# ds2-lab/LambdaFS

Hardware: AMD Instinct MI355X
Metric: RS encode+decode GiB/s device-resident; 1/2/4/8 MI355X; %HBM roofline (higher is better)
Workload: dtype u8; 1 GPU; RS(10,4) encode + 1-erasure decode (data shard 0), 1024 KiB cells, 1024 stripes/GPU, device-resident; encodeBulk / decodeBulk via hrs_encode_dev / hrs_decode_dev; stripes_per_gpu=1024, stripes_total=1024, cell_bytes=1048576, k=10, p=4, parallelism=stripe-sharded x1 (RCCL: matrix broadcast + barriers only)

## Files before the change

include/hrs.h:

```cpp
#ifndef HRS_H_
#define HRS_H_

#include <stddef.h>
#include <stdint.h>

#ifdef __cplusplus
extern "C" {
#endif

typedef int hrs_status;
enum {
  HRS_OK = 0,
  HRS_EINVAL = 1,
  HRS_ETOOMANY = 2,
  HRS_EDEVICE = 3,
  HRS_ENOMEM = 4,
  HRS_EALIGN = 5
};

typedef struct hrs_codec hrs_codec;

enum {
  HRS_CODE_RS = 0,
  HRS_CODE_XOR = 1,
// ... 7 lines not shown
  int device;
  int reserved[7];
} hrs_opts;


hrs_status hrs_create(int stripe_size, int parity_size, const hrs_opts* opts, hrs_codec** out);
hrs_status hrs_create_code(int code, int stripe_size, int parity_size, const hrs_opts* opts,
                           hrs_codec** out);
int hrs_code_kind(const hrs_codec* codec);
hrs_status hrs_create_src(int stripe_size, int parity_size, int src_parity_size, const hrs_opts* opts,
                          hrs_codec** out);
hrs_status hrs_src_layout(const hrs_codec* codec, int* src_parities, int* rs_parities, int* group_degree);
void hrs_destroy(hrs_codec* codec);
const char* hrs_last_error(const hrs_codec* codec);
const char* hrs_last_kernel(const hrs_codec* codec);
const char* hrs_last_host_path(const hrs_codec* codec);
const char* hrs_version(void);


int hrs_device_count(void);
int hrs_codec_device(const hrs_codec* codec);

int hrs_stripe_size(const hrs_codec* codec);
int hrs_parity_size(const hrs_codec* codec);
int hrs_symbol_size(const hrs_codec* codec);


hrs_status hrs_locations_to_read_list(const hrs_codec* codec, const int* erased, int num_erased, int* to_read,
                                      int* num_to_read);

// ... 122 lines not shown
```

lambdafs_amd/_lib.py:

```python
import ctypes
import os

try:
    import torch
except ImportError:
    torch = None

_HERE = os.path.dirname(os.path.abspath(__file__))
LIB_PATH = os.environ.get("HRS_LIB") or os.path.join(_HERE, "libhrs.so")
PROBE_LIB_PATH = os.path.join(_HERE, "libhrs_probe.so")

HRS_OK = 0
HRS_EINVAL = 1
HRS_ETOOMANY = 2
HRS_EDEVICE = 3
HRS_ENOMEM = 4
HRS_EALIGN = 5

HRS_CODE_RS = 0
HRS_CODE_XOR = 1
HRS_CODE_NRS = 2
HRS_CODE_SRC = 3

EXPORTS = (
    "hrs_create", "hrs_create_code", "hrs_create_src", "hrs_src_layout", "hrs_code_kind", "hrs_destroy",
    "hrs_last_error", "hrs_version", "hrs_locations_to_read_list",
    "hrs_stripe_size", "hrs_parity_size", "hrs_symbol_size",
    "hrs_locations_to_read", "hrs_encode_matrix", "hrs_decode_matrix",
    "hrs_encode", "hrs_decode", "hrs_decode3", "hrs_encode_crc", "hrs_decode_crc",
    "hrs_encode_dev", "hrs_decode_dev", "hrs_decode_batch_dev", "hrs_apply_dev", "hrs_crc32_dev",
    "hrs_encode_crc_dev", "hrs_decode_crc_dev", "hrs_decode_batch_host", "hrs_encode_batch_host",
    "hrs_encode_submit", "hrs_decode_submit", "hrs_collect", "hrs_pending", "hrs_ticket_shape",
    "hrs_set_kernel_mode", "hrs_last_kernel", "hrs_wait", "hrs_release",
    "hrs_device_count", "hrs_codec_device", "hrs_decode_batch_host_multi", "hrs_encode_batch_host_multi",
    "hrs_set_timing", "hrs_ticket_gpu_ms", "hrs_last_host_path",
    "hrs_compute_error_locations", "hrs_scrub_dev", "hrs_scrub_batch_host",
    "hrs_heal_dev", "hrs_heal_batch_host", "hrs_heal_host",
)
PROBE_EXPORTS = ("hrs_probe_stream", "hrs_probe_rows")


class HrsError(IOError):

    def __init__(self, status, msg):
        super().__init__(f"hrs status {status}: {msg}")
        self.status = status


class HipOpts(ctypes.Structure):
    _fields_ = [("device", ctypes.c_int), ("reserved", ctypes.c_int * 7)]


# ... 46 lines not shown
        "hrs_encode_batch_host_multi": ([PP, I, P, S, S, S, S], I),
        "hrs_device_count": ([], I),
        "hrs_set_timing": ([P, I], I),
        "hrs_ticket_gpu_ms": ([P, ctypes.c_uint64, ctypes.POINTER(ctypes.c_float)], I),
        "hrs_codec_device": ([P], I),
        "hrs_encode_submit": ([P, PP, S, I, ctypes.POINTER(ctypes.c_uint64)], I),
        "hrs_decode_submit": ([P, PP, IP, I, IP, I, IP, I, S, I, ctypes.POINTER(ctypes.c_uint64)], I),
        "hrs_collect": ([P, ctypes.c_uint64, PP, P], I),
        "hrs_pending": ([P], I),
        "hrs_wait": ([P, ctypes.c_uint64], I),
        "hrs_release": ([P, ctypes.c_uint64], I),
        "hrs_ticket_shape": ([P, ctypes.c_uint64, IP, ctypes.POINTER(ctypes.c_size_t), IP], I),
        "hrs_set_kernel_mode": ([P, I], I),
        "hrs_last_kernel": ([P], ctypes.c_char_p),
        "hrs_last_host_path": ([P], ctypes.c_char_p),
        "hrs_compute_error_locations": ([P, IP, IP, IP, IP], I),
        "hrs_scrub_dev": ([P, PP, S, S, S, P, S, P], I),
        "hrs_scrub_batch_host": ([P, P, S, S, S, S, P, S], I),
        "hrs_heal_dev": ([P, PP, S, S, S, P, S, P], I),
        "hrs_heal_batch_host": ([P, P, S, S, S, S, P, S], I),
        "hrs_heal_host": ([P, PP, S, P], I),
    }
    for name, (args, res) in sigs.items():
        f = getattr(L, name)
        f.argtypes = args
        f.restype = res
    _lib = L
    return L


# ... 39 lines not shown
```

lambdafs_amd/csrc/hrs_api.cpp:

```cpp
#include <hip/hip_runtime.h>

#include <algorithm>
#include <cstdio>
#include <cstring>
#include <map>
#include <string>
#include <vector>

#include "../../include/hrs.h"
#include "hrs_codec.hpp"
#include <cstdarg>

#include "gf256.hpp"

namespace hrs::api {

namespace gf = hrs::gf;

thread_local std::string g_create_error;

hrs_status fail(hrs_codec* c, hrs_status st, const char* fmt, ...) {
  char buf[512];
  va_list ap;
  va_start(ap, fmt);
// ... 118 lines not shown
  if (group_degree) *group_degree = c->src_d;
  return HRS_OK;
}

void hrs_destroy(hrs_codec* c) {
  if (!c) return;
  if (c->device == HRS_DEVICE_NONE) {
    delete c;
    return;
  }
  DeviceGuard g(c->device);
  if (c->stream) {
    (void)hipStreamSynchronize(c->stream);
    (void)hipStreamDestroy(c->stream);
  }
  if (c->crc_tables_a) (void)hipFree(c->crc_tables_a);
  for (auto& kv : c->crc_fold_tables) {
    for (auto& u : kv.second.uses) {
      (void)hipEventSynchronize(u.ev);
      (void)hipEventDestroy(u.ev);
    }
    (void)hipFree(kv.second.dev);
  }
  if (c->crc_raw_done) {
    (void)hipEventSynchronize(c->crc_raw_done);
    (void)hipEventDestroy(c->crc_raw_done);
  }
  if (c->crc_raw) (void)hipFree(c->crc_raw);
  for (auto& h : c->host) {
    if (h.stream) {
// ... 144 lines not shown
```

lambdafs_amd/csrc/hrs_codec.hpp:

```cpp
#pragma once
#include <hip/hip_runtime.h>

#include <cstdint>
#include <map>
#include <set>
#include <string>
#include <vector>

#include "../../include/hrs.h"
#include "crc32.hpp"
#include "hrs_internal.hpp"

namespace hrs {
class CopyPool;
}

struct hrs_codec {
  int kind = HRS_CODE_RS;
  int k = 0;
  int p = 0;
  int n = 0;
  int device = 0;
  int kernel_mode = 0;
  std::vector<uint8_t> g;
// ... 62 lines not shown
    hipStream_t stream = nullptr;
    hipEvent_t done = nullptr;
    hipEvent_t t_start = nullptr;
    hipEvent_t t_end = nullptr;
    bool timed = false;
    bool busy = false;
    bool queued = false;
    uint64_t ticket = 0;
    int nout = 0, nlive = 0, ncrc = 0;
    size_t len = 0, pitch = 0, crc_off = 0;
  } async[hrs::kAsyncSlots];
  uint64_t async_tickets = 0;
  bool timing = false;
  std::string err;
  std::string last_kernel;
  const char* last_host_path = "";
  int numa_node = -2;
};


#pragma GCC visibility push(hidden)
namespace hrs::api {

hrs_status fail(hrs_codec* c, hrs_status st, const char* fmt, ...) __attribute__((format(printf, 3, 4)));
hrs_status hip_fail(hrs_codec* c, hipError_t e, const char* what);

struct DeviceGuard {
  int prev = -1;
  bool ok = true;
  explicit DeviceGuard(int dev) {
    if (dev < 0) {
      ok = false;
      return;
    }
    if (hipGetDevice(&prev) != hipSuccess) {
      ok = false;
      return;
    }
    if (prev != dev && hipSetDevice(dev) != hipSuccess) ok = false;
  }
  ~DeviceGuard() {
    int cur = -1;
    if (prev >= 0 && hipGetDevice(&cur) == hipSuccess && cur != prev) (void)hipSetDevice(prev);
  }
};

inline bool aligned16(const void* p) { return (reinterpret_cast<uintptr_t>(p) & 15u) == 0; }

bool zero_copy_on();
unsigned zero_copy_blocks();
bool runtime_pinned(const void* p, size_t len);
bool host_device_ptr(const void* p, size_t len, uint8_t** dp);
hrs::CopyPool& copy_pool(hrs_codec* c);
uint8_t host_store_mode();

inline bool static_encode_family(const hrs_codec* c) { return c->kind == HRS_CODE_RS || c->kind == HRS_CODE_NRS; }

bool decode_locations_ok(const hrs_codec* c, const int* erased, int ne, const int* to_read, int nr, const int* ntr,
                         int nn);
// ... 3 lines not shown
hrs_status build_decode_matrix(hrs_codec* c, const int* erased, int ne, const int* ntr, int nn, int zero_ntr,
                               std::vector<uint8_t>& d);
hrs_status build_nrs_decode_matrix(hrs_codec* c, int ne, const int* ntr, int nn, std::vector<uint8_t>& d);
const std::vector<uint8_t>* cached_decode_matrix(hrs_codec* c, const int* erased, int ne, const int* ntr, int nn,
                                                 int zero_ntr, hrs_status* st);
std::vector<int> src_neighbors(const hrs_codec* c, int loc);
void src_params(int k, int p, int s_in, int* s, int* r, int* d);
hrs_status src_locations(hrs_codec* c, const int* erased, int ne, std::vector<int>& out);
hrs_status decode5_matrix(hrs_codec* c, const int* erased, int ne, const int* ntr, int nn,
                          const uint8_t* const* rows, std::vector<uint8_t>& tmp, const uint8_t** out,
                          const int* to_read = nullptr, int nr = -1);
void init_encode_matrix(hrs_codec* c);

hrs_status run_apply(hrs_codec* c, const uint8_t* m, int nout, int nin, const uint8_t* const* in_rows,
                     size_t in_stride, uint8_t* const* out_rows, size_t out_stride, size_t len, size_t nstripes,
                     hipStream_t s, bool static_kp);
size_t crc_raw_bytes_for(size_t len, size_t nstripes, int nrows);
hrs_status run_crc(hrs_codec* c, const uint8_t* const* rows, const size_t* strides, int nrows, size_t len,
                   size_t nstripes, const uint32_t* crc_in, uint32_t* crc_out, hipStream_t s, uint32_t* raw);
hrs_status encode_crc_impl(hrs_codec* c, const uint8_t* const* in_rows, size_t in_stride, uint8_t* const* out_rows,
                           size_t out_stride, size_t len, size_t nstripes, const uint32_t* crc_in, uint32_t* crc_out,
                           hipStream_t s, uint32_t* raw, uint64_t* host_fold_win = nullptr);
hrs_status apply_crc_impl(hrs_codec* c, const uint8_t* m, int nout, int nin, const uint8_t* const* in_rows,
                          size_t in_stride, uint8_t* const* out_rows, size_t out_stride, size_t len, size_t nstripes,
                          const uint32_t* crc_in, uint32_t* crc_out, hipStream_t s, uint32_t* raw,
                          uint64_t* host_fold_win = nullptr);
bool encode_crc_one_pass(const hrs_codec* c, size_t len, size_t nstripes);
bool apply_crc_one_pass(const hrs_codec* c, int nout, int nlive, size_t len);

hrs_status scrub_code_ok(hrs_codec* c, size_t report_stride, bool with_reports);
hrs_status run_scrub(hrs_codec* c, const uint8_t* const* rows, size_t stride, size_t len, size_t nstripes,
// ... 6 lines not shown
```

lambdafs_amd/csrc/hrs_dispatch.cpp:

```cpp
#include <hip/hip_runtime.h>

#include <algorithm>
#include <cstdio>
#include <cstdlib>
#include <cstring>
#include <map>
#include <string>
#include <vector>

#include "../../include/hrs.h"
#include "hrs_codec.hpp"
#include "crc32.hpp"
#include "hrs_crc.hpp"
#include "hrs_internal.hpp"

namespace hrs::api {

using hrs::RowArgs;

hrs_status run_apply(hrs_codec* c, const uint8_t* m, int nout, int nin, const uint8_t* const* in_rows,
                     size_t in_stride, uint8_t* const* out_rows, size_t out_stride, size_t len,
                     size_t nstripes, hipStream_t s, bool static_kp) {
  if (nout < 0 || nin < 0 || nout > 255 || nin > 255) return fail(c, HRS_EINVAL, "bad matrix shape %dx%d", nout, nin);
  if (nout == 0 || len == 0 || nstripes == 0) return HRS_OK;
  for (int o = 0; o < nout; ++o)
    if (!out_rows[o]) return fail(c, HRS_EINVAL, "output row %d is NULL", o);
  std::vector<int> live;
  for (int i = 0; i < nin; ++i) {
    bool any = false;
    for (int o = 0; o < nout; ++o) any |= m[o * nin + i] != 0;
    if (any) {
      if (!in_rows[i]) return fail(c, HRS_EINVAL, "input row %d is NULL but has nonzero coefficients", i);
      live.push_back(i);
    }
  }
  if (static_cast<int>(live.size()) != nin || !static_encode_family(c) || m != c->g.data()) static_kp = false;
  bool vec_ok = (in_stride % 16 == 0) && (out_stride % 16 == 0);
  for (int i : live) vec_ok &= aligned16(in_rows[i]);
  for (int o = 0; o < nout; ++o) vec_ok &= aligned16(out_rows[o]);
  const int mode = c->kernel_mode;
  if (mode == 2) vec_ok = false;
  if (mode == 1 || mode == 2) static_kp = false;

  const uint64_t nwin = vec_ok ? len / hrs::kWindowBytes : 0;
  const uint64_t tail_off = nwin * hrs::kWindowBytes;
  const uint64_t tail = len - tail_off;

  if (live.empty()) {
    for (int o = 0; o < nout; ++o)
      for (size_t st = 0; st < nstripes; ++st) {
        hipError_t e = hipMemsetAsync(out_rows[o] + st * out_stride, 0, len, s);
        if (e != hipSuccess) return hip_fail(c, e, "hipMemsetAsync");
      }
    c->last_kernel.clear();
// ... 1 lines not shown
  }

  if (static_kp && nwin > 0) {
    RowArgs a{};
    for (int i = 0; i < nin; ++i) a.in[i] = in_rows[i];
    for (int o = 0; o < nout; ++o) a.out[o] = out_rows[o];
    a.in_stride = in_stride;
    a.out_stride = out_stride;
    a.len = len;
    a.nwin = nwin;
    a.ntasks = nwin * nstripes;
    a.nin = nin;
    a.nout = nout;
    bool handled = false;
    const int family = c->kind == HRS_CODE_NRS ? hrs::kStaticCauchy : hrs::kStaticRs;
    hipError_t e = hrs::launch_static_encode(family, c->k, c->p, a, s, &handled);
    if (e != hipSuccess) return hip_fail(c, e, "static encode launch");
    if (handled) {
      c->last_kernel = hrs::last_kernel();
      if (tail == 0) return HRS_OK;
      std::vector<const uint8_t*> tin(nin);
      std::vector<uint8_t*> tout(nout);
      for (int i = 0; i < nin; ++i) tin[i] = in_rows[i] + tail_off;
      for (int o = 0; o < nout; ++o) tout[o] = out_rows[o] + tail_off;
      const std::string main_kernel = c->last_kernel;
      const hrs_status st =
          run_apply(c, m, nout, nin, tin.data(), in_stride, tout.data(), out_stride, tail, nstripes, s, false);
      c->last_kernel = main_kernel;
      return st;
    }
  }

  const int nlive = static_cast<int>(live.size());
  bool all_ones = (nout == 1) && nwin > 0 && mode == 0;
  for (int i : live) all_ones &= m[i] == 1;
  if (all_ones) {
    for (int i0 = 0; i0 < nlive; i0 += hrs::kMaxInRuntime) {
      const int ni = std::min(hrs::kMaxInRuntime, nlive - i0);
      RowArgs a{};
      for (int i = 0; i < ni; ++i) a.in[i] = in_rows[live[i0 + i]];
      a.out[0] = out_rows[0];
      a.in_stride = in_stride;
// ... 39 lines not shown
      RowArgs a{};
      for (int i = 0; i < ni; ++i) a.in[i] = in_rows[live[i0 + i]];
      for (int o = 0; o < no; ++o) {
        a.out[o] = out_rows[o0 + o];
        for (int i = 0; i < ni; ++i) hrs::set_coef(a, o, i, m[(o0 + o) * nin + live[i0 + i]]);
      }
      a.in_stride = in_stride;
      a.out_stride = out_stride;
      a.nin = ni;
      a.nout = no;
      a.accumulate = i0 > 0;
      if (nwin > 0) {
        a.len = len;
        a.nwin = nwin;
        a.ntasks = nwin * nstripes;
        hipError_t e = stream ? hrs::launch_bitsliced_stream(a, s) : hrs::launch_bitsliced(a, s);
        if (e != hipSuccess) return hip_fail(c, e, "bitsliced launch");
        c->last_kernel = hrs::last_kernel();
      }
      if (tail > 0) {
        RowArgs b = a;
        for (int i = 0; i < ni; ++i) b.in[i] = a.in[i] + tail_off;
        for (int o = 0; o < no; ++o) b.out[o] = a.out[o] + tail_off;
        b.len = tail;
        b.nwin = 0;
        b.ntasks = tail * nstripes;
        hipError_t e = hrs::launch_bytewise(b, s);
        if (e != hipSuccess) return hip_fail(c, e, "bytewise launch");
        if (nwin == 0) c->last_kernel = hrs::last_kernel();
      }
    }
  }
  return HRS_OK;
}


hrs_status upload(hrs_codec* c, const std::vector<uint32_t>& h, uint32_t** out) {
  hipError_t e = hipMalloc(out, h.size() * 4);
  if (e != hipSuccess) return fail(c, HRS_ENOMEM, "hipMalloc: %s", hipGetErrorString(e));
  e = hipMemcpy(*out, h.data(), h.size() * 4, hipMemcpyHostToDevice);
  if (e != hipSuccess) return hip_fail(c, e, "hipMemcpy tables");
  return HRS_OK;
}

// ... 344 lines not shown
  DeviceGuard g(c->device);
  if (!g.ok) return fail(c, HRS_EDEVICE, "cannot select HIP device %d", c->device);
  hipStream_t s = static_cast<hipStream_t>(stream);
  hrs_status st = crc_scratch(c, crc_raw_bytes_for(len, nstripes, c->n), s);
  if (st != HRS_OK) return st;
  return crc_scratch_release(
      c, s, encode_crc_impl(c, in_rows, in_stride, out_rows, out_stride, len, nstripes, crc_in, crc_out, s, c->crc_raw));
}

hrs_status hrs_encode_dev(hrs_codec* c, const uint8_t* const* in_rows, size_t in_stride, uint8_t* const* out_rows,
                          size_t out_stride, size_t len, size_t nstripes, void* stream) {
  if (!c) return HRS_EINVAL;
  if (!in_rows || !out_rows) return fail(c, HRS_EINVAL, "row arrays are NULL");
  DeviceGuard g(c->device);
  if (!g.ok) return fail(c, HRS_EDEVICE, "cannot select HIP device %d", c->device);
  return run_apply(c, c->g.data(), c->p, c->k, in_rows, in_stride, out_rows, out_stride, len, nstripes,
                   static_cast<hipStream_t>(stream), static_encode_family(c));
}

hrs_status hrs_decode_dev(hrs_codec* c, const uint8_t* const* rows, size_t in_stride, uint8_t* const* out_rows,
                          size_t out_stride, const int* erased, int ne, const int* ntr, int nn, size_t len,
                          size_t nstripes, void* stream) {
  if (!c) return HRS_EINVAL;
  if (!rows || ne < 0 || nn < 0 || (ne > 0 && (!out_rows || !erased)) || (nn > 0 && !ntr))
    return fail(c, HRS_EINVAL, "bad decode arguments");
  if (ne == 0 && c->kind == HRS_CODE_RS) return HRS_OK;
  std::vector<uint8_t> tmp;
  const uint8_t* d = nullptr;
  hrs_status st = decode5_matrix(c, erased, ne, ntr, nn, rows, tmp, &d);
  if (st != HRS_OK) return st;
  DeviceGuard g(c->device);
  if (!g.ok) return fail(c, HRS_EDEVICE, "cannot select HIP device %d", c->device);
  return run_apply(c, d, ne, c->n, rows, in_stride, out_rows, out_stride, len, nstripes,
                   static_cast<hipStream_t>(stream), false);
}

hrs_status hrs_decode_crc_dev(hrs_codec* c, const uint8_t* const* rows, size_t in_stride, uint8_t* const* out_rows,
                              size_t out_stride, const int* erased, int ne, const int* ntr, int nn, size_t len,
                              size_t nstripes, const uint32_t* crc_in, uint32_t* crc_out, void* stream) {
  if (!c) return HRS_EINVAL;
  if (!rows || ne < 0 || nn < 0 || (ne > 0 && (!out_rows || !erased || !crc_out)) || (nn > 0 && !ntr))
    return fail(c, HRS_EINVAL, "bad decode arguments");
  if (ne == 0 || nstripes == 0) return HRS_OK;
  std::vector<uint8_t> tmp;
  const uint8_t* d = nullptr;
  hrs_status st = decode5_matrix(c, erased, ne, ntr, nn, rows, tmp, &d);
  if (st != HRS_OK) return st;
  DeviceGuard g(c->device);
  if (!g.ok) return fail(c, HRS_EDEVICE, "cannot select HIP device %d", c->device);
  hipStream_t s = static_cast<hipStream_t>(stream);
  st = crc_scratch(c, crc_raw_bytes_for(len, nstripes, ne), s);
  if (st != HRS_OK) return st;
  return crc_scratch_release(c, s, apply_crc_impl(c, d, ne, c->n, rows, in_stride, out_rows, out_stride, len, nstripes,
                                                  crc_in, crc_out, s, c->crc_raw));
}

hrs_status hrs_apply_dev(hrs_codec* c, const uint8_t* m, int nout, int nin, const uint8_t* const* in_rows,
                         size_t in_stride, uint8_t* const* out_rows, size_t out_stride, size_t len, size_t nstripes,
                         void* stream) {
  if (!c) return HRS_EINVAL;
  if (!m || !in_rows || !out_rows || nout < 1 || nin < 1 || nout > 255 || nin > 255)
    return fail(c, HRS_EINVAL, "bad apply arguments");
  DeviceGuard g(c->device);
  if (!g.ok) return fail(c, HRS_EDEVICE, "cannot select HIP device %d", c->device);
  return run_apply(c, m, nout, nin, in_rows, in_stride, out_rows, out_stride, len, nstripes,
                   static_cast<hipStream_t>(stream), false);
}

}
```

lambdafs_amd/csrc/hrs_internal.hpp:

```cpp
#pragma once
#include <cstddef>
#include <cstdint>
#include <hip/hip_runtime.h>

namespace hrs {

constexpr int kMaxIn = 32;
constexpr int kMaxInRuntime = 16;
constexpr int kMaxInRuntimeWide = 8;
inline int runtime_in_chunk(int nout) { return nout <= 5 ? kMaxInRuntime : kMaxInRuntimeWide; }
constexpr int kMaxOut = 8;

constexpr int kWindowBytes = 2048;
constexpr int kBlockThreads = 256;
constexpr int kWavesPerBlock = kBlockThreads / 64;

struct RowArgs {
  const uint8_t* in[kMaxIn];
  uint8_t* out[kMaxOut];
  uint64_t cw[kMaxIn];
  uint64_t in_stride;
  uint64_t out_stride;
  uint64_t len;
  uint64_t nwin;
// ... 2 lines not shown
  int nout;
  int accumulate;
  int order;
};

inline void set_coef(RowArgs& a, int o, int i, uint8_t v) {
  a.cw[i] = (a.cw[i] & ~(0xFFull << (8 * o))) | (static_cast<uint64_t>(v) << (8 * o));
}

enum class KernelKind : int {
  kStaticEncode = 0,
  kBitsliced = 1,
  kBytewise = 2,
};

enum { kStaticRs = 0, kStaticCauchy = 1 };
hipError_t launch_static_encode(int family, int k, int p, const RowArgs& a, hipStream_t s, bool* handled);
hipError_t launch_bitsliced(const RowArgs& a, hipStream_t s);
hipError_t launch_bitsliced_stream(const RowArgs& a, hipStream_t s);
hipError_t launch_bytewise(const RowArgs& a, hipStream_t s);
hipError_t launch_xor(const RowArgs& a, hipStream_t s);
int device_cu_count();

void note_kernel(const char* name);
const char* last_kernel();


constexpr int kBatchMaxIn = 32;
constexpr int kHostBatchSlots = 3;
constexpr int kAsyncSlots = 4;
constexpr int kHostSlots = 8;
struct BatchPlan {
  int nin;
  int nout;
// ... 52 lines not shown
```

lambdafs_amd/csrc/hrs_kernels.hip:

```cpp
#include <hip/hip_runtime.h>

#include <cstdlib>
#include <string>

#include "hrs_device.hpp"
#include "hrs_launch.hpp"

namespace hrs {
namespace {


__constant__ gf::Tables d_tables = gf::make_tables();


template <int K, int P, class MATRIX>
__device__ __forceinline__ void encode_static_body(const RowArgs& a) {
  const int lane = threadIdx.x & 63;
  const WaveTasks wt = wave_tasks(a.ntasks, a.order);
  for (uint32_t j = 0; j < 0xFFFFFFFFu; ++j) {
    const uint64_t t = wt.at(j);
    if (t >= wt.end) break;
    const uint64_t stripe = t / a.nwin;
    const uint64_t off = (t - stripe * a.nwin) * kWindowBytes;
    uint32_t acc[P][8];
// ... 95 lines not shown
      if (x == 0) continue;
      const int lx = s_log[x];
#pragma unroll
      for (int o = 0; o < kMaxOut; ++o) {
        const uint8_t c = static_cast<uint8_t>(a.cw[r] >> (8 * o));
        if (o < a.nout && c != 0) acc[o] ^= s_exp[lx + s_log[c]];
      }
    }
#pragma unroll
    for (int o = 0; o < kMaxOut; ++o)
      if (o < a.nout) a.out[o][stripe * a.out_stride + col] = acc[o];
  }
}

template <int K, int P>
hipError_t launch_static(const RowArgs& a, hipStream_t s) {
  auto kern = encode_static_kernel<K, P>;
  note_kernel_t("encode_static_kernel", K, P);
  const unsigned g = stream_grid(a.ntasks);
  hipLaunchKernelGGL(kern, dim3(g), dim3(kBlockThreads), 0, s, with_order(a, kOrderStaticEncode));
  return hipGetLastError();
}

template <int K, int P>
hipError_t launch_cauchy(const RowArgs& a, hipStream_t s) {
  auto kern = encode_cauchy_kernel<K, P>;
  note_kernel_t("encode_cauchy_kernel", K, P);
  const unsigned g = stream_grid(a.ntasks);
  hipLaunchKernelGGL(kern, dim3(g), dim3(kBlockThreads), 0, s, with_order(a, kOrderStaticEncode));
  return hipGetLastError();
}

}

int device_cu_count() { return device_cus(); }

namespace {
thread_local std::string t_last_kernel;
}
void note_kernel(const char* name) { t_last_kernel = name; }
const char* last_kernel() { return t_last_kernel.c_str(); }

hipError_t launch_static_encode(int family, int k, int p, const RowArgs& a, hipStream_t s, bool* handled) {
  *handled = true;
  if (family == kStaticCauchy) {
    if (k == 10 && p == 4) return launch_cauchy<10, 4>(a, s);
    if (k == 6 && p == 3) return launch_cauchy<6, 3>(a, s);
    *handled = false;
    return hipSuccess;
  }
  if (k == 10 && p == 4) return launch_static<10, 4>(a, s);
  if (k == 6 && p == 3) return launch_static<6, 3>(a, s);
  if (k == 3 && p == 2) return launch_static<3, 2>(a, s);
  if (k == 12 && p == 4) return launch_static<12, 4>(a, s);
  *handled = false;
  return hipSuccess;
}

template <int NINB>
hipError_t launch_xor_n(const RowArgs& a, hipStream_t s) {
  auto kern = xor_kernel<NINB>;
  note_kernel_t("xor_kernel", NINB);
  hipLaunchKernelGGL(kern, dim3(stream_grid(a.ntasks)), dim3(kBlockThreads), 0, s, with_order(a, kOrderStaticEncode));
  return hipGetLastError();
}

hipError_t launch_xor(const RowArgs& a, hipStream_t s) {
  if (a.nin <= 4) return launch_xor_n<4>(a, s);
  if (a.nin <= 8) return launch_xor_n<8>(a, s);
// ... 14 lines not shown
```

lambdafs_amd/csrc/hrs_launch.hpp:

```cpp
#pragma once
#include <hip/hip_runtime.h>

#include <atomic>
#include <cstdint>
#include <cstdlib>
#include <string>

#include "hrs_internal.hpp"

namespace hrs {

inline void kname_arg(std::string& s, int v) { s += std::to_string(v); }
inline void kname_arg(std::string& s, bool v) { s += v ? "true" : "false"; }
inline void kname_arg(std::string& s, const char* v) { s += v; }
template <typename... T>
inline void note_kernel_t(const char* base, T... v) {
  std::string s(base);
  if constexpr (sizeof...(T) > 0) {
    const char* sep = "<";
    ((s += sep, kname_arg(s, v), sep = ", "), ...);
    s += '>';
  }
  note_kernel(s.c_str());
}
// ... 22 lines not shown

constexpr int kOrderStaticEncode = 1;
constexpr int kOrderRuntime = 1;
constexpr int kOrderBatch = 1;
constexpr int kOrderFusedEncode = 1;
constexpr int kOrderDecodeCrc = 1;
constexpr int kOrderCrc = 1;
constexpr int kOrderScrub = 1;

template <class A>
inline A with_order(A a, int dflt) {
  a.order = task_order(dflt);
  return a;
}

inline int blocks_per_cu(int dflt = 2) {
  static int v = [] {
    const char* e = getenv("HRS_BLOCKS_PER_CU");
    int x = e ? atoi(e) : 0;
    return (x >= 1 && x <= 32) ? x : 0;
  }();
  return v ? v : dflt;
}

inline thread_local unsigned t_grid_cap = 0;

struct GridCap {
  unsigned prev;
  explicit GridCap(unsigned cap) : prev(t_grid_cap) { t_grid_cap = cap; }
  ~GridCap() { t_grid_cap = prev; }
// ... 28 lines not shown
```

lambdafs_amd/csrc/hrs_runtime.hip:

```cpp
#include <hip/hip_runtime.h>

#include <cstdlib>

#include "hrs_device.hpp"
#include "hrs_launch.hpp"

namespace hrs {
namespace {

template <int NOUT, int NINB>
__global__ void __launch_bounds__(kBlockThreads) bitsliced_kernel(const RowArgs a) {
  const int lane = threadIdx.x & 63;
  const WaveTasks wt = wave_tasks(a.ntasks, a.order);
  for (uint32_t j = 0; j < 0xFFFFFFFFu; ++j) {
    const uint64_t t = wt.at(j);
    if (t >= wt.end) break;
    int nin = a.nin;
    asm volatile("" : "+s"(nin));
    const uint64_t stripe = t / a.nwin;
    const uint64_t off = (t - stripe * a.nwin) * kWindowBytes;
    const uint64_t in_base = stripe * a.in_stride + off;
    uint32_t rows[NINB][8];
#pragma unroll
    for (int r = 0; r < NINB; ++r)
// ... 150 lines not shown

constexpr int kStreamGroup = 4;

template <int NOUT, int NINB>
constexpr bool kPipeFits = !BitLoop<NOUT, NINB>::kRolled && 16 * NINB + 8 * NOUT <= 232;

bool use_pipe() {
  static bool v = [] {
    const char* e = getenv("HRS_PIPE");
    return !(e && e[0] == '0');
  }();
  return v;
}

template <int NOUT, int NINB>
hipError_t launch_bits_n(const RowArgs& a, hipStream_t s) {
  auto kern = bitsliced_kernel<NOUT, NINB>;
  const char* name = "bitsliced_kernel";
  if constexpr (kPipeFits<NOUT, NINB>)
    if (use_pipe()) {
      kern = bitsliced_pipe_kernel<NOUT, NINB>;
      name = "bitsliced_pipe_kernel";
    }
  note_kernel_t(name, NOUT, NINB);
  const int per_cu = BitLoop<NOUT, NINB>::kRolled ? 3 : 2;
  hipLaunchKernelGGL(kern, dim3(stream_grid(a.ntasks, per_cu)), dim3(kBlockThreads), 0, s, with_order(a, kOrderRuntime));
  return hipGetLastError();
}

template <int NOUT>
hipError_t launch_bits(const RowArgs& a, hipStream_t s) {
  if (a.nin <= 4) return launch_bits_n<NOUT, 4>(a, s);
  if (a.nin <= 8) return launch_bits_n<NOUT, 8>(a, s);
  if constexpr (NOUT < 6) {
    if (a.nin <= 12) return launch_bits_n<NOUT, 12>(a, s);
    if (a.nin <= 16) return launch_bits_n<NOUT, 16>(a, s);
  }
  return hipErrorInvalidValue;
}

template <int NOUT>
hipError_t launch_stream_n(const RowArgs& a, hipStream_t s) {
  auto kern = bitsliced_stream_kernel<NOUT, kStreamGroup>;
  note_kernel_t("bitsliced_stream_kernel", NOUT, kStreamGroup);
  const int per_cu = NOUT >= 4 ? 3 : 2;
  hipLaunchKernelGGL(kern, dim3(stream_grid(a.ntasks, per_cu)), dim3(kBlockThreads), 0, s, with_order(a, kOrderRuntime));
  return hipGetLastError();
}

}

hipError_t launch_bitsliced_stream(const RowArgs& a, hipStream_t s) {
  if (a.nin < 1 || a.nin > kMaxIn) return hipErrorInvalidValue;
  switch (a.nout) {
    case 1: return launch_stream_n<1>(a, s);
    case 2: return launch_stream_n<2>(a, s);
    case 3: return launch_stream_n<3>(a, s);
    case 4: return launch_stream_n<4>(a, s);
    case 5: return launch_stream_n<5>(a, s);
    case 6: return launch_stream_n<6>(a, s);
    case 7: return launch_stream_n<7>(a, s);
    case 8: return launch_stream_n<8>(a, s);
    default: return hipErrorInvalidValue;
  }
}

hipError_t launch_bitsliced(const RowArgs& a, hipStream_t s) {
  switch (a.nout) {
    case 1: return launch_bits<1>(a, s);
    case 2: return launch_bits<2>(a, s);
    case 3: return launch_bits<3>(a, s);
    case 4: return launch_bits<4>(a, s);
    case 5: return launch_bits<5>(a, s);
    case 6: return launch_bits<6>(a, s);
    case 7: return launch_bits<7>(a, s);
    case 8: return launch_bits<8>(a, s);
    default: return hipErrorInvalidValue;
  }
}

}
```

lambdafs_amd/erasure_code.py:

```python
import abc
import ctypes

import numpy as np

from . import _lib
from ._lib import check, int_array, ptr_array


class TooManyErasedLocations(IOError):
    """io.hops.erasure_coding.TooManyErasedLocations (TooManyErasedLocations.java:26-31)."""


class ErasureCode(abc.ABC):

    @abc.abstractmethod
    def encode(self, message, parity):
        """ErasureCode.java:38 — message: k ints, parity (out): p ints."""

    @abc.abstractmethod
    def decode(self, data, erasedLocations, erasedValues, locationsToRead=None, locationsNotToRead=None):
        """ErasureCode.java:55 (3-arg) and :75 (5-arg)."""

    def locationsToReadForDecode(self, erasedLocations):
        locationsToRead = []
# ... 179 lines not shown
    def locationsToReadForDecode(self, erasedLocations):
        n = self._k + self._p
        buf = (ctypes.c_int * max(1, n))()
        cnt = ctypes.c_int(0)
        erased = [int(e) for e in erasedLocations]
        self._check(_lib.lib().hrs_locations_to_read_list(self._handle(), int_array(erased), len(erased), buf,
                                                           ctypes.byref(cnt)))
        return list(buf[: cnt.value])

    def setKernelMode(self, mode):
        self._check(_lib.lib().hrs_set_kernel_mode(self._handle(), int(mode)))

    def lastKernel(self):
        return _lib.lib().hrs_last_kernel(self._handle()).decode()

    def lastHostPath(self):
        return _lib.lib().hrs_last_host_path(self._handle()).decode()

    def encodeMatrix(self):
        g = np.zeros((self._p, self._k), dtype=np.uint8)
        self._check(_lib.lib().hrs_encode_matrix(self._handle(), g.ctypes.data))
        return g

    def decodeMatrix(self, erasedLocations, locationsNotToRead, zero_not_to_read=True):
        n = self._k + self._p
        d = np.zeros((max(1, len(erasedLocations)), n), dtype=np.uint8)
        self._check(_lib.lib().hrs_decode_matrix(
            self._handle(), int_array(erasedLocations), len(erasedLocations),
            int_array(locationsNotToRead), len(locationsNotToRead), int(bool(zero_not_to_read)),
            d.ctypes.data))
# ... 367 lines not shown
```

Before: 4137 GiB/s.

## Add runtime autotuner that times task-order candidates per launch shape

```diff
diff --git a/include/hrs.h b/include/hrs.h
--- a/include/hrs.h
+++ b/include/hrs.h
@@ -45,6 +45,8 @@
 void hrs_destroy(hrs_codec* codec);
 const char* hrs_last_error(const hrs_codec* codec);
 const char* hrs_last_kernel(const hrs_codec* codec);
+void hrs_order_info(const hrs_codec* codec, int* order, int* state);
+int hrs_order_samples(const hrs_codec* codec, int candidate, int* order, float* ms);
 const char* hrs_last_host_path(const hrs_codec* codec);
 const char* hrs_version(void);
 
diff --git a/lambdafs_amd/_lib.py b/lambdafs_amd/_lib.py
--- a/lambdafs_amd/_lib.py
+++ b/lambdafs_amd/_lib.py
@@ -36,6 +36,7 @@
     "hrs_set_timing", "hrs_ticket_gpu_ms", "hrs_last_host_path",
     "hrs_compute_error_locations", "hrs_scrub_dev", "hrs_scrub_batch_host",
     "hrs_heal_dev", "hrs_heal_batch_host", "hrs_heal_host",
+    "hrs_order_info", "hrs_order_samples",
 )
 PROBE_EXPORTS = ("hrs_probe_stream", "hrs_probe_rows")
 
@@ -112,6 +113,8 @@
         "hrs_set_kernel_mode": ([P, I], I),
         "hrs_last_kernel": ([P], ctypes.c_char_p),
         "hrs_last_host_path": ([P], ctypes.c_char_p),
+        "hrs_order_info": ([P, IP, IP], None),
+        "hrs_order_samples": ([P, I, IP, ctypes.POINTER(ctypes.c_float)], I),
         "hrs_compute_error_locations": ([P, IP, IP, IP, IP], I),
         "hrs_scrub_dev": ([P, PP, S, S, S, P, S, P], I),
         "hrs_scrub_batch_host": ([P, P, S, S, S, S, P, S], I),
diff --git a/lambdafs_amd/csrc/hrs_api.cpp b/lambdafs_amd/csrc/hrs_api.cpp
--- a/lambdafs_amd/csrc/hrs_api.cpp
+++ b/lambdafs_amd/csrc/hrs_api.cpp
@@ -156,6 +156,7 @@
     (void)hipStreamSynchronize(c->stream);
     (void)hipStreamDestroy(c->stream);
   }
+  hrs::order_tune_destroy(c->order_tune);
   if (c->crc_tables_a) (void)hipFree(c->crc_tables_a);
   for (auto& kv : c->crc_fold_tables) {
     for (auto& u : kv.second.uses) {
diff --git a/lambdafs_amd/csrc/hrs_codec.hpp b/lambdafs_amd/csrc/hrs_codec.hpp
--- a/lambdafs_amd/csrc/hrs_codec.hpp
+++ b/lambdafs_amd/csrc/hrs_codec.hpp
@@ -100,6 +100,7 @@
   bool timing = false;
   std::string err;
   std::string last_kernel;
+  hrs::OrderTuneCtx* order_tune = nullptr;
   const char* last_host_path = "";
   int numa_node = -2;
 };
@@ -129,6 +130,17 @@
     int cur = -1;
     if (prev >= 0 && hipGetDevice(&cur) == hipSuccess && cur != prev) (void)hipSetDevice(prev);
   }
+};
+
+struct OrderTuneScope {
+  hrs::OrderTuneCtx* t;
+  bool prev;
+  explicit OrderTuneScope(hrs_codec* c) {
+    if (!c->order_tune) c->order_tune = hrs::order_tune_create();
+    t = c->order_tune;
+    prev = hrs::order_tune_enable(t, true);
+  }
+  ~OrderTuneScope() { hrs::order_tune_enable(t, prev); }
 };
 
 inline bool aligned16(const void* p) { return (reinterpret_cast<uintptr_t>(p) & 15u) == 0; }
@@ -162,7 +174,7 @@
 
 hrs_status run_apply(hrs_codec* c, const uint8_t* m, int nout, int nin, const uint8_t* const* in_rows,
                      size_t in_stride, uint8_t* const* out_rows, size_t out_stride, size_t len, size_t nstripes,
-                     hipStream_t s, bool static_kp);
+                     hipStream_t s, bool static_kp, bool tail_of_static = false);
 size_t crc_raw_bytes_for(size_t len, size_t nstripes, int nrows);
 hrs_status run_crc(hrs_codec* c, const uint8_t* const* rows, const size_t* strides, int nrows, size_t len,
                    size_t nstripes, const uint32_t* crc_in, uint32_t* crc_out, hipStream_t s, uint32_t* raw);
diff --git a/lambdafs_amd/csrc/hrs_dispatch.cpp b/lambdafs_amd/csrc/hrs_dispatch.cpp
--- a/lambdafs_amd/csrc/hrs_dispatch.cpp
+++ b/lambdafs_amd/csrc/hrs_dispatch.cpp
@@ -20,7 +20,7 @@
 
 hrs_status run_apply(hrs_codec* c, const uint8_t* m, int nout, int nin, const uint8_t* const* in_rows,
                      size_t in_stride, uint8_t* const* out_rows, size_t out_stride, size_t len,
-                     size_t nstripes, hipStream_t s, bool static_kp) {
+                     size_t nstripes, hipStream_t s, bool static_kp, bool tail_of_static) {
   if (nout < 0 || nin < 0 || nout > 255 || nin > 255) return fail(c, HRS_EINVAL, "bad matrix shape %dx%d", nout, nin);
   if (nout == 0 || len == 0 || nstripes == 0) return HRS_OK;
   for (int o = 0; o < nout; ++o)
@@ -38,6 +38,8 @@
   bool vec_ok = (in_stride % 16 == 0) && (out_stride % 16 == 0);
   for (int i : live) vec_ok &= aligned16(in_rows[i]);
   for (int o = 0; o < nout; ++o) vec_ok &= aligned16(out_rows[o]);
+  if (!c->order_tune) c->order_tune = hrs::order_tune_create();
+  hrs::OrderTuneCtx* const tune = c->order_tune;
   const int mode = c->kernel_mode;
   if (mode == 2) vec_ok = false;
   if (mode == 1 || mode == 2) static_kp = false;
@@ -69,7 +71,7 @@
     a.nout = nout;
     bool handled = false;
     const int family = c->kind == HRS_CODE_NRS ? hrs::kStaticCauchy : hrs::kStaticRs;
-    hipError_t e = hrs::launch_static_encode(family, c->k, c->p, a, s, &handled);
+    hipError_t e = hrs::launch_static_encode(family, c->k, c->p, a, s, &handled, tune);
     if (e != hipSuccess) return hip_fail(c, e, "static encode launch");
     if (handled) {
       c->last_kernel = hrs::last_kernel();
@@ -80,7 +82,7 @@
       for (int o = 0; o < nout; ++o) tout[o] = out_rows[o] + tail_off;
       const std::string main_kernel = c->last_kernel;
       const hrs_status st =
-          run_apply(c, m, nout, nin, tin.data(), in_stride, tout.data(), out_stride, tail, nstripes, s, false);
+          run_apply(c, m, nout, nin, tin.data(), in_stride, tout.data(), out_stride, tail, nstripes, s, false, true);
       c->last_kernel = main_kernel;
       return st;
     }
@@ -150,7 +152,7 @@
         a.len = len;
         a.nwin = nwin;
         a.ntasks = nwin * nstripes;
-        hipError_t e = stream ? hrs::launch_bitsliced_stream(a, s) : hrs::launch_bitsliced(a, s);
+        hipError_t e = stream ? hrs::launch_bitsliced_stream(a, s, tune) : hrs::launch_bitsliced(a, s, tune);
         if (e != hipSuccess) return hip_fail(c, e, "bitsliced launch");
         c->last_kernel = hrs::last_kernel();
       }
@@ -163,7 +165,10 @@
         b.ntasks = tail * nstripes;
         hipError_t e = hrs::launch_bytewise(b, s);
         if (e != hipSuccess) return hip_fail(c, e, "bytewise launch");
-        if (nwin == 0) c->last_kernel = hrs::last_kernel();
+        if (nwin == 0) {
+          c->last_kernel = hrs::last_kernel();
+          if (!tail_of_static) hrs::order_note_none(tune);
+        }
       }
     }
   }
@@ -538,6 +543,7 @@
   if (!in_rows || !out_rows) return fail(c, HRS_EINVAL, "row arrays are NULL");
   DeviceGuard g(c->device);
   if (!g.ok) return fail(c, HRS_EDEVICE, "cannot select HIP device %d", c->device);
+  OrderTuneScope tuning(c);
   return run_apply(c, c->g.data(), c->p, c->k, in_rows, in_stride, out_rows, out_stride, len, nstripes,
                    static_cast<hipStream_t>(stream), static_encode_family(c));
 }
@@ -555,6 +561,7 @@
   if (st != HRS_OK) return st;
   DeviceGuard g(c->device);
   if (!g.ok) return fail(c, HRS_EDEVICE, "cannot select HIP device %d", c->device);
+  OrderTuneScope tuning(c);
   return run_apply(c, d, ne, c->n, rows, in_stride, out_rows, out_stride, len, nstripes,
                    static_cast<hipStream_t>(stream), false);
 }
@@ -579,6 +586,14 @@
                                                   crc_in, crc_out, s, c->crc_raw));
 }
 
+void hrs_order_info(const hrs_codec* c, int* order, int* state) {
+  hrs::order_info(c ? c->order_tune : nullptr, order, state);
+}
+
+int hrs_order_samples(const hrs_codec* c, int candidate, int* order, float* ms) {
+  return hrs::order_samples(c ? c->order_tune : nullptr, candidate, order, ms);
+}
+
 hrs_status hrs_apply_dev(hrs_codec* c, const uint8_t* m, int nout, int nin, const uint8_t* const* in_rows,
                          size_t in_stride, uint8_t* const* out_rows, size_t out_stride, size_t len, size_t nstripes,
                          void* stream) {
@@ -587,6 +602,7 @@
     return fail(c, HRS_EINVAL, "bad apply arguments");
   DeviceGuard g(c->device);
   if (!g.ok) return fail(c, HRS_EDEVICE, "cannot select HIP device %d", c->device);
+  OrderTuneScope tuning(c);
   return run_apply(c, m, nout, nin, in_rows, in_stride, out_rows, out_stride, len, nstripes,
                    static_cast<hipStream_t>(stream), false);
 }
diff --git a/lambdafs_amd/csrc/hrs_internal.hpp b/lambdafs_amd/csrc/hrs_internal.hpp
--- a/lambdafs_amd/csrc/hrs_internal.hpp
+++ b/lambdafs_amd/csrc/hrs_internal.hpp
@@ -40,10 +40,26 @@
   kBytewise = 2,
 };
 
+struct OrderTuneCtx;
+struct OrderPick {
+  int order;
+  int state;
+  int trial;
+};
+OrderTuneCtx* order_tune_create();
+void order_tune_destroy(OrderTuneCtx* t);
+bool order_tune_enable(OrderTuneCtx* t, bool on);
+OrderPick order_begin(OrderTuneCtx* t, int family, int dflt, const RowArgs& a, hipStream_t s);
+void order_end(OrderTuneCtx* t, const OrderPick& pk, hipStream_t s, bool launched);
+void order_note_none(OrderTuneCtx* t);
+void order_info(const OrderTuneCtx* t, int* order, int* state);
+int order_samples(const OrderTuneCtx* t, int cand, int* order, float* ms);
+
 enum { kStaticRs = 0, kStaticCauchy = 1 };
-hipError_t launch_static_encode(int family, int k, int p, const RowArgs& a, hipStream_t s, bool* handled);
-hipError_t launch_bitsliced(const RowArgs& a, hipStream_t s);
-hipError_t launch_bitsliced_stream(const RowArgs& a, hipStream_t s);
+hipError_t launch_static_encode(int family, int k, int p, const RowArgs& a, hipStream_t s, bool* handled,
+                                OrderTuneCtx* tune = nullptr);
+hipError_t launch_bitsliced(const RowArgs& a, hipStream_t s, OrderTuneCtx* tune = nullptr);
+hipError_t launch_bitsliced_stream(const RowArgs& a, hipStream_t s, OrderTuneCtx* tune = nullptr);
 hipError_t launch_bytewise(const RowArgs& a, hipStream_t s);
 hipError_t launch_xor(const RowArgs& a, hipStream_t s);
 int device_cu_count();
diff --git a/lambdafs_amd/csrc/hrs_kernels.hip b/lambdafs_amd/csrc/hrs_kernels.hip
--- a/lambdafs_amd/csrc/hrs_kernels.hip
+++ b/lambdafs_amd/csrc/hrs_kernels.hip
@@ -133,21 +133,17 @@
 }
 
 template <int K, int P>
-hipError_t launch_static(const RowArgs& a, hipStream_t s) {
+hipError_t launch_static(const RowArgs& a, hipStream_t s, OrderTuneCtx* t) {
   auto kern = encode_static_kernel<K, P>;
   note_kernel_t("encode_static_kernel", K, P);
-  const unsigned g = stream_grid(a.ntasks);
-  hipLaunchKernelGGL(kern, dim3(g), dim3(kBlockThreads), 0, s, with_order(a, kOrderStaticEncode));
-  return hipGetLastError();
+  return launch_tuned(kern, stream_grid(a.ntasks), a, s, t, kTuneStaticEncode, kOrderStaticEncode);
 }
 
 template <int K, int P>
-hipError_t launch_cauchy(const RowArgs& a, hipStream_t s) {
+hipError_t launch_cauchy(const RowArgs& a, hipStream_t s, OrderTuneCtx* t) {
   auto kern = encode_cauchy_kernel<K, P>;
   note_kernel_t("encode_cauchy_kernel", K, P);
-  const unsigned g = stream_grid(a.ntasks);
-  hipLaunchKernelGGL(kern, dim3(g), dim3(kBlockThreads), 0, s, with_order(a, kOrderStaticEncode));
-  return hipGetLastError();
+  return launch_tuned(kern, stream_grid(a.ntasks), a, s, t, kTuneStaticEncode, kOrderStaticEncode);
 }
 
 }
@@ -160,18 +156,19 @@
 void note_kernel(const char* name) { t_last_kernel = name; }
 const char* last_kernel() { return t_last_kernel.c_str(); }
 
-hipError_t launch_static_encode(int family, int k, int p, const RowArgs& a, hipStream_t s, bool* handled) {
+hipError_t launch_static_encode(int family, int k, int p, const RowArgs& a, hipStream_t s, bool* handled,
+                                OrderTuneCtx* t) {
   *handled = true;
   if (family == kStaticCauchy) {
-    if (k == 10 && p == 4) return launch_cauchy<10, 4>(a, s);
-    if (k == 6 && p == 3) return launch_cauchy<6, 3>(a, s);
+    if (k == 10 && p == 4) return launch_cauchy<10, 4>(a, s, t);
+    if (k == 6 && p == 3) return launch_cauchy<6, 3>(a, s, t);
     *handled = false;
     return hipSuccess;
   }
-  if (k == 10 && p == 4) return launch_static<10, 4>(a, s);
-  if (k == 6 && p == 3) return launch_static<6, 3>(a, s);
-  if (k == 3 && p == 2) return launch_static<3, 2>(a, s);
-  if (k == 12 && p == 4) return launch_static<12, 4>(a, s);
+  if (k == 10 && p == 4) return launch_static<10, 4>(a, s, t);
+  if (k == 6 && p == 3) return launch_static<6, 3>(a, s, t);
+  if (k == 3 && p == 2) return launch_static<3, 2>(a, s, t);
+  if (k == 12 && p == 4) return launch_static<12, 4>(a, s, t);
   *handled = false;
   return hipSuccess;
 }
diff --git a/lambdafs_amd/csrc/hrs_launch.hpp b/lambdafs_amd/csrc/hrs_launch.hpp
--- a/lambdafs_amd/csrc/hrs_launch.hpp
+++ b/lambdafs_amd/csrc/hrs_launch.hpp
@@ -7,6 +7,7 @@
 #include <string>
 
 #include "hrs_internal.hpp"
+#include "hrs_order_tune.hpp"
 
 namespace hrs {
 
@@ -60,6 +61,17 @@
   return a;
 }
 
+template <class Kern>
+inline hipError_t launch_tuned(Kern kern, unsigned grid, RowArgs a, hipStream_t s, OrderTuneCtx* t, int family,
+                               int dflt) {
+  const OrderPick pk = order_begin(t, family, dflt, a, s);
+  a.order = pk.order;
+  hipLaunchKernelGGL(kern, dim3(grid), dim3(kBlockThreads), 0, s, a);
+  const hipError_t e = hipGetLastError();
+  order_end(t, pk, s, e == hipSuccess);
+  return e;
+}
+
 inline int blocks_per_cu(int dflt = 2) {
   static int v = [] {
     const char* e = getenv("HRS_BLOCKS_PER_CU");
diff --git a/lambdafs_amd/csrc/hrs_order_launch.cpp b/lambdafs_amd/csrc/hrs_order_launch.cpp
--- /dev/null
+++ b/lambdafs_amd/csrc/hrs_order_launch.cpp
@@ -0,0 +1,179 @@
+#include <hip/hip_runtime.h>
+
+#include <cstdlib>
+
+#include "hrs_launch.hpp"
+#include "hrs_order_tune.hpp"
+
+namespace hrs {
+
+constexpr uint64_t kTuneMinBytes = 7ull << 29;
+
+constexpr int kTunePool = 16;
+
+struct OrderTuneCtx {
+  OrderTuner core;
+  struct Slot {
+    hipEvent_t a = nullptr, b = nullptr;
+    bool busy = false, ended = false;
+    OrderKey key{};
+    int cand = 0;
+  } pool[kTunePool];
+  bool enabled = false;
+  int last_order = -1, last_state = kTuneBypassed;
+  bool has_key = false;
+  OrderKey last_key{};
+};
+
+OrderTuneCtx* order_tune_create() { return new OrderTuneCtx(); }
+
+void order_tune_destroy(OrderTuneCtx* t) {
+  if (!t) return;
+  for (auto& s : t->pool) {
+    if (s.a) (void)hipEventDestroy(s.a);
+    if (s.b) (void)hipEventDestroy(s.b);
+  }
+  delete t;
+}
+
+bool order_tune_enable(OrderTuneCtx* t, bool on) {
+  const bool prev = t->enabled;
+  t->enabled = on;
+  return prev;
+}
+
+void order_note_none(OrderTuneCtx* t) {
+  if (!t) return;
+  t->last_order = -1;
+  t->last_state = kTuneBypassed;
+  t->has_key = false;
+}
+
+void order_info(const OrderTuneCtx* t, int* order, int* state) {
+  if (order) *order = t ? t->last_order : -1;
+  if (state) *state = t ? t->last_state : kTuneBypassed;
+}
+
+int order_samples(const OrderTuneCtx* t, int cand, int* order, float* ms) {
+  if (!t || !t->has_key || cand < 0 || cand >= kTuneCandidates) return 0;
+  if (order) *order = kTuneOrders[t->last_key.family][cand];
+  return t->core.samples(t->last_key, cand, ms);
+}
+
+namespace {
+
+bool env_is_zero(const char* name) {
+  const char* e = getenv(name);
+  return e && e[0] == '0' && e[1] == 0;
+}
+
+uint64_t min_bytes() {
+  const char* e = getenv("HRS_ORDER_TUNE_MIN_BYTES");
+  return (e && *e) ? strtoull(e, nullptr, 10) : kTuneMinBytes;
+}
+
+void release(OrderTuneCtx::Slot& s) { s.busy = s.ended = false; }
+
+void harvest(OrderTuneCtx* t, const OrderKey* only) {
+  bool dirty = false;
+  for (auto& s : t->pool) {
+    if (!s.busy || !s.ended) continue;
+    hipError_t e;
+    if (only && !(s.key < *only) && !(*only < s.key))
+      e = hipEventSynchronize(s.b);
+    else
+      e = hipEventQuery(s.b);
+    if (e == hipErrorNotReady) {
+      dirty = true;
+      continue;
+    }
+    float ms = 0.f;
+    if (e == hipSuccess) e = hipEventElapsedTime(&ms, s.a, s.b);
+    if (e == hipSuccess) {
+      t->core.sample(s.key, s.cand, ms);
+    } else {
+      dirty = true;
+      t->core.fail(s.key);
+    }
+    release(s);
+  }
+  if (dirty) (void)hipGetLastError();
+}
+
+}
+
+OrderPick order_begin(OrderTuneCtx* t, int family, int dflt, const RowArgs& a, hipStream_t s) {
+  OrderPick pk{task_order(dflt), kTuneBypassed, -1};
+  if (!t) return pk;
+  t->last_order = pk.order;
+  t->last_state = kTuneBypassed;
+  t->has_key = false;
+  const char* forced = getenv("HRS_TASK_ORDER");
+  if (!t->enabled || t_grid_cap != 0 || (forced && *forced) || env_is_zero("HRS_ORDER_TUNE")) return pk;
+  const uint64_t bytes = a.ntasks * kWindowBytes * static_cast<uint64_t>(a.nin + a.nout);
+  if (a.nwin == 0 || bytes < min_bytes()) return pk;
+  hipStreamCaptureStatus cap = hipStreamCaptureStatusNone;
+  if (hipStreamIsCapturing(s, &cap) != hipSuccess || cap != hipStreamCaptureStatusNone) {
+    (void)hipGetLastError();
+    return pk;
+  }
+  const OrderKey key{family, a.nin, a.nout, a.len, a.ntasks / a.nwin, a.in_stride, a.out_stride};
+  t->has_key = true;
+  t->last_key = key;
+  harvest(t, nullptr);
+  OrderTuner::Pick p = t->core.next(key);
+  if (p.state == kTuneCalibrating && p.cand < 0 && t->core.waiting(key) && !env_is_zero("HRS_ORDER_TUNE_WAIT")) {
+    harvest(t, &key);
+    p = t->core.next(key);
+  }
+  pk.order = p.order;
+  pk.state = p.state;
+  if (p.cand >= 0) {
+    OrderTuneCtx::Slot* slot = nullptr;
+    for (auto& x : t->pool)
+      if (!x.busy) {
+        slot = &x;
+        break;
+      }
+    hipError_t e = hipSuccess;
+    if (slot && !slot->a) e = hipEventCreate(&slot->a);
+    if (slot && !slot->b && e == hipSuccess) e = hipEventCreate(&slot->b);
+    if (slot && e == hipSuccess) e = hipEventRecord(slot->a, s);
+    if (!slot) {
+      pk.order = dflt;
+    } else if (e != hipSuccess) {
+      (void)hipGetLastError();
+      t->core.fail(key);
+      pk.order = dflt;
+      pk.state = kTuneFrozen;
+    } else {
+      slot->busy = true;
+      slot->ended = false;
+      slot->key = key;
+      slot->cand = p.cand;
+      pk.trial = static_cast<int>(slot - t->pool);
+    }
+  }
+  t->last_order = pk.order;
+  t->last_state = pk.state;
+  return pk;
+}
+
+void order_end(OrderTuneCtx* t, const OrderPick& pk, hipStream_t s, bool launched) {
+  if (!t || pk.trial < 0) return;
+  OrderTuneCtx::Slot& slot = t->pool[pk.trial];
+  if (!launched) {
+    release(slot);
+    return;
+  }
+  if (hipEventRecord(slot.b, s) != hipSuccess) {
+    (void)hipGetLastError();
+    t->core.fail(slot.key);
+    release(slot);
+    return;
+  }
+  slot.ended = true;
+  t->core.issued(slot.key, slot.cand);
+}
+
+}
diff --git a/lambdafs_amd/csrc/hrs_order_tune.cpp b/lambdafs_amd/csrc/hrs_order_tune.cpp
--- /dev/null
+++ b/lambdafs_amd/csrc/hrs_order_tune.cpp
@@ -0,0 +1,86 @@
+#include "hrs_order_tune.hpp"
+
+#include <algorithm>
+
+namespace hrs {
+
+OrderTuner::Pick OrderTuner::next(const OrderKey& key) {
+  const int dflt = kTuneOrders[key.family][0];
+  auto it = map_.find(key);
+  if (it == map_.end()) {
+    if (map_.size() >= kTuneMaxKeys) map_.clear();
+    it = map_.emplace(key, Entry{}).first;
+  }
+  Entry& e = it->second;
+  if (e.frozen) return {e.order, kTuneFrozen, -1};
+  if (!e.cold_done) {
+    e.cold_done = true;
+    return {dflt, kTuneCalibrating, -1};
+  }
+  int cand = 0;
+  for (int c = 1; c < kTuneCandidates; ++c)
+    if (e.issued[c] < e.issued[cand]) cand = c;
+  if (e.issued[cand] < kTuneRepeats) return {kTuneOrders[key.family][cand], kTuneCalibrating, cand};
+  return {dflt, kTuneCalibrating, -1};
+}
+
+void OrderTuner::issued(const OrderKey& key, int cand) {
+  auto it = map_.find(key);
+  if (it == map_.end() || cand < 0 || cand >= kTuneCandidates) return;
+  if (it->second.issued[cand] < kTuneRepeats) ++it->second.issued[cand];
+}
+
+void OrderTuner::sample(const OrderKey& key, int cand, float ms) {
+  auto it = map_.find(key);
+  if (it == map_.end() || cand < 0 || cand >= kTuneCandidates) return;
+  Entry& e = it->second;
+  if (e.frozen || e.got[cand] >= e.issued[cand]) return;
+  e.ms[cand][e.got[cand]++] = ms;
+  for (int c = 0; c < kTuneCandidates; ++c)
+    if (e.got[c] < kTuneRepeats) return;
+  decide(key, e);
+}
+
+void OrderTuner::decide(const OrderKey& key, Entry& e) {
+  float lo[kTuneCandidates], med[kTuneCandidates], hi[kTuneCandidates];
+  for (int c = 0; c < kTuneCandidates; ++c) {
+    float s[kTuneRepeats];
+    std::copy(e.ms[c], e.ms[c] + kTuneRepeats, s);
+    std::sort(s, s + kTuneRepeats);
+    lo[c] = s[0];
+    med[c] = s[kTuneRepeats / 2];
+    hi[c] = s[kTuneRepeats - 1];
+  }
+  int best = 0;
+  for (int c = 1; c < kTuneCandidates; ++c) {
+    const bool clears = med[c] * 100.0f < med[0] * static_cast<float>(100 - kTuneMarginPct);
+    const bool apart = hi[c] < lo[0];
+    if (clears && apart && (best == 0 || med[c] < med[best])) best = c;
+  }
+  e.frozen = true;
+  e.order = kTuneOrders[key.family][best];
+}
+
+void OrderTuner::fail(const OrderKey& key) {
+  auto it = map_.find(key);
+  if (it == map_.end()) return;
+  it->second.frozen = true;
+  it->second.order = kTuneOrders[key.family][0];
+}
+
+bool OrderTuner::waiting(const OrderKey& key) const {
+  auto it = map_.find(key);
+  if (it == map_.end() || it->second.frozen) return false;
+  for (int c = 0; c < kTuneCandidates; ++c)
+    if (it->second.got[c] < it->second.issued[c]) return true;
+  return false;
+}
+
+int OrderTuner::samples(const OrderKey& key, int cand, float* ms) const {
+  auto it = map_.find(key);
+  if (it == map_.end() || cand < 0 || cand >= kTuneCandidates) return 0;
+  for (int i = 0; i < kTuneRepeats; ++i) ms[i] = it->second.ms[cand][i];
+  return it->second.got[cand];
+}
+
+}
diff --git a/lambdafs_amd/csrc/hrs_order_tune.hpp b/lambdafs_amd/csrc/hrs_order_tune.hpp
--- /dev/null
+++ b/lambdafs_amd/csrc/hrs_order_tune.hpp
@@ -0,0 +1,60 @@
+#pragma once
+#include <cstddef>
+#include <cstdint>
+#include <map>
+#include <tuple>
+
+namespace hrs {
+
+constexpr int kTuneRepeats = 3;
+constexpr int kTuneCandidates = 2;
+constexpr int kTuneMarginPct = 2;
+constexpr size_t kTuneMaxKeys = 64;
+
+enum { kTuneBypassed = 0, kTuneCalibrating = 1, kTuneFrozen = 2 };
+
+enum { kTuneStaticEncode = 0, kTuneRuntime = 1 };
+constexpr int kTuneOrders[2][kTuneCandidates] = {
+    {1, 0},
+    {1, 2},
+};
+
+struct OrderKey {
+  int family, nin, nout;
+  uint64_t len, nstripes, in_stride, out_stride;
+  bool operator<(const OrderKey& o) const {
+    return std::tie(family, nin, nout, len, nstripes, in_stride, out_stride) <
+           std::tie(o.family, o.nin, o.nout, o.len, o.nstripes, o.in_stride, o.out_stride);
+  }
+};
+
+class OrderTuner {
+ public:
+  struct Pick {
+    int order;
+    int state;
+    int cand;
+  };
+  Pick next(const OrderKey& key);
+  void issued(const OrderKey& key, int cand);
+  void sample(const OrderKey& key, int cand, float ms);
+  void fail(const OrderKey& key);
+
+  bool waiting(const OrderKey& key) const;
+  size_t keys() const { return map_.size(); }
+  int samples(const OrderKey& key, int cand, float* ms) const;
+
+ private:
+  struct Entry {
+    bool cold_done = false;
+    bool frozen = false;
+    int order = 0;
+    int issued[kTuneCandidates] = {};
+    int got[kTuneCandidates] = {};
+    float ms[kTuneCandidates][kTuneRepeats] = {};
+  };
+  void decide(const OrderKey& key, Entry& e);
+  std::map<OrderKey, Entry> map_;
+};
+
+}
diff --git a/lambdafs_amd/csrc/hrs_runtime.hip b/lambdafs_amd/csrc/hrs_runtime.hip
--- a/lambdafs_amd/csrc/hrs_runtime.hip
+++ b/lambdafs_amd/csrc/hrs_runtime.hip
@@ -188,7 +188,7 @@
 }
 
 template <int NOUT, int NINB>
-hipError_t launch_bits_n(const RowArgs& a, hipStream_t s) {
+hipError_t launch_bits_n(const RowArgs& a, hipStream_t s, OrderTuneCtx* t) {
   auto kern = bitsliced_kernel<NOUT, NINB>;
   const char* name = "bitsliced_kernel";
   if constexpr (kPipeFits<NOUT, NINB>)
@@ -198,57 +198,55 @@
     }
   note_kernel_t(name, NOUT, NINB);
   const int per_cu = BitLoop<NOUT, NINB>::kRolled ? 3 : 2;
-  hipLaunchKernelGGL(kern, dim3(stream_grid(a.ntasks, per_cu)), dim3(kBlockThreads), 0, s, with_order(a, kOrderRuntime));
-  return hipGetLastError();
+  return launch_tuned(kern, stream_grid(a.ntasks, per_cu), a, s, t, kTuneRuntime, kOrderRuntime);
 }
 
 template <int NOUT>
-hipError_t launch_bits(const RowArgs& a, hipStream_t s) {
-  if (a.nin <= 4) return launch_bits_n<NOUT, 4>(a, s);
-  if (a.nin <= 8) return launch_bits_n<NOUT, 8>(a, s);
+hipError_t launch_bits(const RowArgs& a, hipStream_t s, OrderTuneCtx* t) {
+  if (a.nin <= 4) return launch_bits_n<NOUT, 4>(a, s, t);
+  if (a.nin <= 8) return launch_bits_n<NOUT, 8>(a, s, t);
   if constexpr (NOUT < 6) {
-    if (a.nin <= 12) return launch_bits_n<NOUT, 12>(a, s);
-    if (a.nin <= 16) return launch_bits_n<NOUT, 16>(a, s);
+    if (a.nin <= 12) return launch_bits_n<NOUT, 12>(a, s, t);
+    if (a.nin <= 16) return launch_bits_n<NOUT, 16>(a, s, t);
   }
   return hipErrorInvalidValue;
 }
 
 template <int NOUT>
-hipError_t launch_stream_n(const RowArgs& a, hipStream_t s) {
+hipError_t launch_stream_n(const RowArgs& a, hipStream_t s, OrderTuneCtx* t) {
   auto kern = bitsliced_stream_kernel<NOUT, kStreamGroup>;
   note_kernel_t("bitsliced_stream_kernel", NOUT, kStreamGroup);
   const int per_cu = NOUT >= 4 ? 3 : 2;
-  hipLaunchKernelGGL(kern, dim3(stream_grid(a.ntasks, per_cu)), dim3(kBlockThreads), 0, s, with_order(a, kOrderRuntime));
-  return hipGetLastError();
-}
-
-}
-
-hipError_t launch_bitsliced_stream(const RowArgs& a, hipStream_t s) {
+  return launch_tuned(kern, stream_grid(a.ntasks, per_cu), a, s, t, kTuneRuntime, kOrderRuntime);
+}
+
+}
+
+hipError_t launch_bitsliced_stream(const RowArgs& a, hipStream_t s, OrderTuneCtx* t) {
   if (a.nin < 1 || a.nin > kMaxIn) return hipErrorInvalidValue;
   switch (a.nout) {
-    case 1: return launch_stream_n<1>(a, s);
-    case 2: return launch_stream_n<2>(a, s);
-    case 3: return launch_stream_n<3>(a, s);
-    case 4: return launch_stream_n<4>(a, s);
-    case 5: return launch_stream_n<5>(a, s);
-    case 6: return launch_stream_n<6>(a, s);
-    case 7: return launch_stream_n<7>(a, s);
-    case 8: return launch_stream_n<8>(a, s);
+    case 1: return launch_stream_n<1>(a, s, t);
+    case 2: return launch_stream_n<2>(a, s, t);
+    case 3: return launch_stream_n<3>(a, s, t);
+    case 4: return launch_stream_n<4>(a, s, t);
+    case 5: return launch_stream_n<5>(a, s, t);
+    case 6: return launch_stream_n<6>(a, s, t);
+    case 7: return launch_stream_n<7>(a, s, t);
+    case 8: return launch_stream_n<8>(a, s, t);
     default: return hipErrorInvalidValue;
   }
 }
 
-hipError_t launch_bitsliced(const RowArgs& a, hipStream_t s) {
+hipError_t launch_bitsliced(const RowArgs& a, hipStream_t s, OrderTuneCtx* t) {
   switch (a.nout) {
-    case 1: return launch_bits<1>(a, s);
-    case 2: return launch_bits<2>(a, s);
-    case 3: return launch_bits<3>(a, s);
-    case 4: return launch_bits<4>(a, s);
-    case 5: return launch_bits<5>(a, s);
-    case 6: return launch_bits<6>(a, s);
-    case 7: return launch_bits<7>(a, s);
-    case 8: return launch_bits<8>(a, s);
+    case 1: return launch_bits<1>(a, s, t);
+    case 2: return launch_bits<2>(a, s, t);
+    case 3: return launch_bits<3>(a, s, t);
+    case 4: return launch_bits<4>(a, s, t);
+    case 5: return launch_bits<5>(a, s, t);
+    case 6: return launch_bits<6>(a, s, t);
+    case 7: return launch_bits<7>(a, s, t);
+    case 8: return launch_bits<8>(a, s, t);
     default: return hipErrorInvalidValue;
   }
 }
diff --git a/lambdafs_amd/erasure_code.py b/lambdafs_amd/erasure_code.py
--- a/lambdafs_amd/erasure_code.py
+++ b/lambdafs_amd/erasure_code.py
@@ -217,6 +217,16 @@
     def lastKernel(self):
         return _lib.lib().hrs_last_kernel(self._handle()).decode()
 
+    def orderInfo(self):
+        order, state = ctypes.c_int(-1), ctypes.c_int(0)
+        _lib.lib().hrs_order_info(self._handle(), ctypes.byref(order), ctypes.byref(state))
+        return order.value, state.value
+
+    def orderSamples(self, candidate):
+        order, ms = ctypes.c_int(-1), (ctypes.c_float * 3)()
+        n = _lib.lib().hrs_order_samples(self._handle(), int(candidate), ctypes.byref(order), ms)
+        return order.value, [float(ms[i]) for i in range(n)]
+
     def lastHostPath(self):
         return _lib.lib().hrs_last_host_path(self._handle()).decode()
 
```

Result: no change. 4140 GiB/s (median of 5 runs) (+0.1%).
